# autonomousvision/unimatch

Hardware: AMD Instinct MI355X
Metric: image_pairs_per_sec (higher is better)
Workload: dtype f16x2

## Files before the change

### unimatch_amd/csrc/conv.hip

```cpp
#include <cstdlib>
#include <cstring>
#ifndef UM_CONV_2P
#define UM_CONV_2P 0
#endif
#include "common.h"
#include "planes.h"

struct ConvArgs {
    const unsigned short* ap;
    long a_plane_stride;
    unsigned row_stride;
    unsigned zero_row;
    const unsigned short* wp;
    long w_plane_stride;
    const float* bias;
    float* out;
    unsigned short* outp;
    long outp_plane_stride;
    int out_ld, out_coff, outp_ld, outp_coff;
    int act;
    int gate, gate_c, gate_zld;
    float* gate_h;
    const float* gate_z;
    float* gate_hout;
    int gate_hout_ld;
    float* stats;
    const float* addend;
    int addend_ld;
    int addend_period;
    int B, Hi, Wi, Cin, Ho, Wo, Cout;
    int KH, KW, stride, pad_h, pad_w;
    int M;
    float out_scale;
    int xcd;
    const float* xf;
    const float* nstats;
    int norm_relu;
};

__device__ __forceinline__ void conv_dma16(const void* base, unsigned byte_off, const unsigned char* lds_dst) {
    const unsigned dst = __builtin_amdgcn_readfirstlane(
        (unsigned)(unsigned long)(const __attribute__((address_space(3))) unsigned char*)lds_dst);
    unsigned keep;
    asm volatile("s_mov_b32 %0, m0\n\ts_mov_b32 m0, %3\n\ts_nop 0\n\tglobal_load_lds_dwordx4 %1, %2\n\ts_mov_b32 m0, %0"
                 : "=&s"(keep)
                 : "v"(byte_off), "s"(base), "s"(dst)
                 : "memory");
}

template <int V>
struct IntC {
    static constexpr int value = V;
};

template <typename T, int NS, int NT, int NT0, int NTP, int WSTRIDE, bool ADDEND>
__device__ __forceinline__ void conv_epilogue_pass(const ConvArgs& a, f32x16 (&acc)[NT], unsigned char* lds, unsigned char* scratch,
                                                   int bt, int rloc0, int nvalid, int part0, bool dense_parts, int n0, int tid,
                                                   int wave, int lane, int half) {
    const int P = a.Ho * a.Wo;
    constexpr int ROWB = 32 * NTP * 4;
    const int nb = n0 + 32 * NT0;
    unsigned char* stg = lds + wave * WSTRIDE;
    const int tl = lane & 31;
    constexpr int CPR = 8 * NTP;
    constexpr int ITER = 32 * CPR / 64;
    constexpr int BATCH = ITER < 4 ? ITER : 4, NBATCH = ITER / BATCH, NSIDE = NT == 4 ? 2 : 1;
    static_assert(ITER % BATCH == 0, "batches cover the iterations");
    const long rowbase = (long)bt * P + rloc0;
    const int nrows = nvalid;
    const int gate = a.gate;
    float* hbase = gate ? a.gate_h + rowbase * a.gate_c : nullptr;
    const float* zbase = gate == 2 ? a.gate_z + rowbase * a.gate_zld : nullptr;
    const float* abase = ADDEND && a.addend ? a.addend + rowbase * a.addend_ld : nullptr;
    const long aback = ADDEND && a.addend_period ? (long)bt * P * a.addend_ld : 0L;
    float* hobase = gate == 2 ? a.gate_hout + rowbase * a.gate_hout_ld : nullptr;
    f32x4 ad[NSIDE][BATCH], gz[NSIDE][BATCH], gh[NSIDE][BATCH];
    auto preload = [&](int b, int slot) {
        if (!abase && !gate) return;
#pragma unroll
        for (int j = 0; j < BATCH; ++j) {
            const int idx = (b * BATCH + j) * 64 + lane;
            const int r = idx / CPR, c = idx - r * CPR;
            const int col = nb + 4 * c;
            if (r < nrows && col < a.Cout) {
                if (abase) ad[slot][j] = *reinterpret_cast<const f32x4*>(abase - aback + (unsigned)(r * a.addend_ld + col));
                if (gate == 1 && col >= a.gate_c) gh[slot][j] = *reinterpret_cast<const f32x4*>(hbase + (unsigned)(r * a.gate_c + col - a.gate_c));
                if (gate == 2) {
                    gz[slot][j] = *reinterpret_cast<const f32x4*>(zbase + (unsigned)(r * a.gate_zld + col));
                    gh[slot][j] = *reinterpret_cast<const f32x4*>(hbase + (unsigned)(r * a.gate_c + col));
                }
            }
        }
    };
    preload(0, 0);
    auto to_lds = [&](auto act_tag, auto bias_tag) {
        constexpr int ACT = decltype(act_tag)::value;
        constexpr bool BIAS = decltype(bias_tag)::value != 0;
#pragma unroll
        for (int nt = 0; nt < NTP; ++nt)
#pragma unroll
            for (int g = 0; g < 4; ++g) {
                const int n = nb + 32 * nt + 8 * g + 4 * half;
                f32x4 v;
#pragma unroll
                for (int i = 0; i < 4; ++i) v[i] = acc[NT0 + nt][4 * g + i] * a.out_scale;
                if (BIAS) v = v + *reinterpret_cast<const f32x4*>(a.bias + min(n, a.Cout - 4));
#pragma unroll
                for (int i = 0; i < 4; ++i) {
                    if (ACT == 1) v[i] = fmaxf(v[i], 0.f);
                    else if (ACT == 2) v[i] = 1.0f / (1.0f + __expf(-v[i]));
                    else if (ACT == 3) v[i] = tanhf(v[i]);
                }
                const int c = 8 * nt + 2 * g + half;
                *reinterpret_cast<f32x4*>(stg + tl * ROWB + ((c ^ (tl & 7)) << 4)) = v;
            }
    };
    auto to_lds_b = [&](auto act_tag) {
        if (a.bias) to_lds(act_tag, IntC<1>{});
        else to_lds(act_tag, IntC<0>{});
    };
    switch (ADDEND && a.addend ? 0 : a.act) {
        case 0: to_lds_b(IntC<0>{}); break;
        case 1: to_lds_b(IntC<1>{}); break;
        case 2: to_lds_b(IntC<2>{}); break;
        default: to_lds_b(IntC<3>{}); break;
    }
    __builtin_amdgcn_wave_barrier();
    if (a.stats) {
        constexpr int RG = 64 / CPR >= 8 ? 8 : 64 / CPR >= 4 ? 4 : 2;
        constexpr int RPG = 32 / RG;
        const int nv = nvalid;
        const int c = lane % CPR, rg = lane / CPR;
        const f32x4 k = *reinterpret_cast<const f32x4*>(stg + (c << 4));
        f32x4 s1 = {0.f, 0.f, 0.f, 0.f}, s2 = {0.f, 0.f, 0.f, 0.f};
        if (rg < RG) {
            if (nv == 32) {
#pragma unroll
                for (int j = 0; j < RPG; ++j) {
                    const int r = rg * RPG + j;
                    const f32x4 d = *reinterpret_cast<const f32x4*>(stg + r * ROWB + ((c ^ (r & 7)) << 4)) - k;
                    s1 = s1 + d;
                    s2 = s2 + d * d;
                }
            } else {
#pragma unroll
                for (int j = 0; j < RPG; ++j) {
                    const int r = rg * RPG + j;
                    f32x4 d = *reinterpret_cast<const f32x4*>(stg + r * ROWB + ((c ^ (r & 7)) << 4)) - k;
                    if (r >= nv) d = f32x4{0.f, 0.f, 0.f, 0.f};
                    s1 = s1 + d;
                    s2 = s2 + d * d;
                }
            }
        }
#pragma unroll
        for (int step = CPR * RG / 2; step >= CPR; step >>= 1)
#pragma unroll
            for (int i = 0; i < 4; ++i) {
                s1[i] += __shfl_down(s1[i], step, 64);
                s2[i] += __shfl_down(s2[i], step, 64);
            }
        float* ws = reinterpret_cast<float*>(scratch) + wave * (2 * 32 * NT) + 32 * NT0;
        float* cnt = reinterpret_cast<float*>(scratch) + 8 * (2 * 32 * NT);
        if (lane == 0) cnt[wave] = (float)nv;
        if (lane < CPR) {
            const float inv = nv > 0 ? 1.0f / (float)nv : 0.f;
            *reinterpret_cast<f32x4*>(ws + 4 * c) = k + s1 * inv;
            *reinterpret_cast<f32x4*>(ws + 32 * NT + 4 * c) = s2 - s1 * s1 * inv;
        }
        __syncthreads();
        const int grp = tid >> 8, gt = tid & 255;
        if (gt < 32 * NTP && nb + gt < a.Cout && (cnt[4 * grp] > 0.f || dense_parts)) {
            const float* w0 = reinterpret_cast<const float*>(scratch) + grp * 4 * (2 * 32 * NT) + 32 * NT0;
            float mean = w0[gt], m2 = w0[32 * NT + gt];
            float n = cnt[4 * grp];
#pragma unroll
            for (int wv = 1; wv < 4; ++wv) {
                const float nw = cnt[4 * grp + wv];
                if (nw > 0.f) {
                    const float mw = w0[wv * (2 * 32 * NT) + gt], m2w = w0[wv * (2 * 32 * NT) + 32 * NT + gt];
                    const float delta = mw - mean, nn = n + nw;
                    mean += delta * (nw / nn);
                    m2 += m2w + delta * delta * (n * nw / nn);
                    n = nn;
                }
            }
            float* pr = a.stats + ((long)(part0 + grp) * 3) * a.Cout + nb + gt;
            pr[0] = n > 0.f ? mean : 0.f;
            pr[a.Cout] = n;
            pr[2 * a.Cout] = n > 0.f ? m2 : 0.f;
        }
    }
    auto store_rows = [&](auto gate_tag, auto add_tag) {
        constexpr int GATE = decltype(gate_tag)::value;
        constexpr bool ADD = decltype(add_tag)::value != 0;
        float* obase = a.out ? a.out + rowbase * a.out_ld + a.out_coff : nullptr;
        unsigned short* pbase = a.outp ? a.outp + rowbase * a.outp_ld + a.outp_coff : nullptr;
#pragma unroll
        for (int b = 0; b < NBATCH; ++b) {
            const int slot = NSIDE == 2 ? (b & 1) : 0;
            if ((ADD || GATE != 0) && NSIDE == 2 && b + 1 < NBATCH) preload(b + 1, (b + 1) & 1);
            if ((ADD || GATE != 0) && NSIDE == 1 && b > 0) preload(b, 0);
#pragma unroll
            for (int j = 0; j < BATCH; ++j) {
                const int idx = (b * BATCH + j) * 64 + lane;
                const int r = idx / CPR, c = idx - r * CPR;
                f32x4 d = *reinterpret_cast<const f32x4*>(stg + r * ROWB + ((c ^ (r & 7)) << 4));
                int col = nb + 4 * c;
                if (r < nrows && col < a.Cout) {
                    if (ADD) {
                        d = d + ad[slot][j];
#pragma unroll
                        for (int i = 0; i < 4; ++i) {
                            if (a.act == 1) d[i] = fmaxf(d[i], 0.f);
                            else if (a.act == 2) d[i] = 1.0f / (1.0f + __expf(-d[i]));
                            else if (a.act == 3) d[i] = tanhf(d[i]);
                        }
                    }
                    bool to_out = obase != nullptr, to_planes = pbase != nullptr;
                    if (GATE == 1) {
                        if (col >= a.gate_c) {
                            col -= a.gate_c;
                            d = d * gh[slot][j];
                            to_out = false;
                        } else {
                            to_planes = false;
                        }
                    } else if (GATE == 2) {
#pragma unroll
                        for (int i = 0; i < 4; ++i) d[i] = (1.0f - gz[slot][j][i]) * gh[slot][j][i] + gz[slot][j][i] * d[i];
                        *reinterpret_cast<f32x4*>(hobase + (unsigned)(r * a.gate_hout_ld + col)) = d;
                    }
                    if (to_out) __builtin_nontemporal_store(d, reinterpret_cast<f32x4*>(obase + (unsigned)(r * a.out_ld + col)));
                    if (to_planes) {
                        unsigned short* dst = pbase + (unsigned)(r * a.outp_ld + col);
                        const unsigned h0 = T::pack2(d[0], d[1]), h1 = T::pack2(d[2], d[3]);
                        *reinterpret_cast<u32x2*>(dst) = u32x2{h0, h1};
                        if (NS == 2) {
                            const f32x2 u0 = T::unpack2(h0), u1 = T::unpack2(h1);
                            const u32x2 lo = u32x2{T::pack2(d[0] - u0[0], d[1] - u0[1]), T::pack2(d[2] - u1[0], d[3] - u1[1])};
                            *reinterpret_cast<u32x2*>(dst + a.outp_plane_stride) = lo;
                        }
                    }
                }
            }
        }
    };
    auto store_rows_g = [&](auto gate_tag) {
        if (ADDEND && a.addend) store_rows(gate_tag, IntC<1>{});
        else store_rows(gate_tag, IntC<0>{});
    };
    if (a.gate == 0) store_rows_g(IntC<0>{});
    else if (a.gate == 1) store_rows_g(IntC<1>{});
    else store_rows_g(IntC<2>{});
}

template <typename T, int NS, int NT, int NTE = NT, bool ADDEND = true>
__device__ __forceinline__ void conv_epilogue(const ConvArgs& a, f32x16 (&acc)[NT], unsigned char* lds, unsigned char* scratch,
                                              int bt, int rloc0, int nvalid, int part0, bool dense_parts, int n0, int tid, int wave,
                                              int lane, int half) {
    constexpr int NP = NTE < NT ? NTE : NT;
    constexpr int WSTRIDE = 32 * (32 * NP * 4);
    conv_epilogue_pass<T, NS, NT, 0, NP, WSTRIDE, ADDEND>(a, acc, lds, scratch, bt, rloc0, nvalid, part0, dense_parts, n0, tid, wave, lane, half);
    if constexpr (NTE < NT)
        conv_epilogue_pass<T, NS, NT, NTE, NT - NTE, WSTRIDE, ADDEND>(a, acc, lds, scratch, bt, rloc0, nvalid, part0, dense_parts, n0, tid, wave,
                                                              lane, half);
}

struct ConvEntryArgs {
    const float* u;
    const float* ustats;
    const unsigned short* sp;
    long s_plane_stride;
    const unsigned short* wp2;
    long w2_plane_stride;
    const float* bias2;
    float* out2;
    float* stats2;
};

template <int NS, int NT>
struct ConvLds {
    static constexpr int TILE = 128 * 64;
    static constexpr int WTILE = 32 * NT * 64;
    static constexpr int STAGE = NS * (TILE + WTILE);
    static constexpr int EPI = 4 * 32 * (32 * NT * 4);
    static constexpr int RING = (2 * STAGE > EPI) ? 2 * STAGE : EPI;
    static constexpr int TOTAL = RING + 8 * 2 * 32 * NT * 4 + 64;
    static constexpr int ENTRY_CIN = 128;
    static constexpr int ENTRY_TOTAL = TOTAL + 2 * ENTRY_CIN * 4;
};

template <typename T, int NS, int NT, bool ENTRY>
__device__ __forceinline__ void conv_body(const ConvArgs& a, const ConvEntryArgs& e, unsigned char* lds) {
    using L = ConvLds<NS, NT>;
    constexpr int TILE = L::TILE, WTILE = L::WTILE, STAGE = L::STAGE, RING = L::RING;

    const int tid = threadIdx.x, lane = tid & 63;
    const int wave = __builtin_amdgcn_readfirstlane(tid >> 6);
    const int half = lane >> 5;
    const int P = a.Ho * a.Wo, tpi = (P + 127) / 128;
    const int ny = (a.Cout + 32 * NT - 1) / (32 * NT);
    const int wg = a.xcd ? xcd_remap(blockIdx.x, gridDim.x) : blockIdx.x;
    const int tile = wg / ny;
    const int bt = tile / tpi, pl0 = (tile - bt * tpi) * 128;
    const int n0 = (wg - tile * ny) * (32 * NT);
    const int cpt = a.Cin >> 5;
    const int nstage = a.KH * a.KW * cpt;
    const int ktot = a.KH * a.KW * a.Cin;

    const int dcp = lane & 3;
    int py[2], px[2], pbase[2];
    bool pok[2];
#pragma unroll
    for (int i = 0; i < 2; ++i) {
        const int p = pl0 + 32 * wave + 16 * i + (lane >> 2);
        pok[i] = p < P;
        const int rem = pok[i] ? p : 0;
        const int y = rem / a.Wo, x = rem - y * a.Wo;
        py[i] = y * a.stride - a.pad_h;
        px[i] = x * a.stride - a.pad_w;
        pbase[i] = bt * a.Hi * a.Wi;
    }
    const unsigned zero_row = a.zero_row;
    unsigned rowoff[2];
    auto set_tap = [&](int ky, int kx) {
#pragma unroll
        for (int i = 0; i < 2; ++i) {
            const int iy = py[i] + ky, ix = px[i] + kx;
            const bool ok = pok[i] && (unsigned)iy < (unsigned)a.Hi && (unsigned)ix < (unsigned)a.Wi;
            if constexpr (ENTRY) {
                rowoff[i] = ok ? (unsigned)(pbase[i] + iy * a.Wi + ix) : ~0u;
            } else {
                const unsigned row = ok ? (unsigned)(pbase[i] + iy * a.Wi + ix) : zero_row;
                rowoff[i] = row * a.row_stride;
            }
        }
    };
    int ky = 0, kx = 0, cc = 0;
    auto stage_async = [&](int c0, int kglob, unsigned char* buf) {
        if constexpr (!ENTRY) {
#pragma unroll
            for (int i = 0; i < 2; ++i) {
                const int r = 32 * wave + 16 * i + (lane >> 2);
                const int sc = dcp ^ ((r >> 2) & 3);
                const unsigned off = rowoff[i] + (unsigned)((c0 + 8 * sc) * 2);
#pragma unroll
                for (int pl = 0; pl < NS; ++pl) conv_dma16(a.ap + pl * a.a_plane_stride, off, buf + pl * TILE + (32 * wave + 16 * i) * 64);
            }
        }
#pragma unroll
        for (int i = 0; i < (2 * NT + 3) / 4; ++i) {
            const int j = wave + 4 * i;
            if (j < 2 * NT) {
                const int r = 16 * j + (lane >> 2);
                const int sc = dcp ^ ((r >> 2) & 3);
                const int n = min(n0 + r, a.Cout - 1);
                const unsigned off = (unsigned)(((long)n * ktot + kglob + 8 * sc) * 2);
#pragma unroll
                for (int pl = 0; pl < NS; ++pl)
                    conv_dma16(a.wp + pl * a.w_plane_stride, off, buf + NS * TILE + pl * WTILE + (16 * j) * 64);
            }
        }
    };
    const int esc = dcp ^ ((lane >> 4) & 3);
    float* sstat = reinterpret_cast<float*>(lds + L::TOTAL);
    f32x4 eu[2][2];
    u32x4 esh[2], esl[2];
    bool eok[2];
    int ec0 = 0;
    auto entry_load = [&](int c0) {
        ec0 = c0 + 8 * esc;
#pragma unroll
        for (int i = 0; i < 2; ++i) {
            eok[i] = rowoff[i] != ~0u;
            const unsigned el = (eok[i] ? rowoff[i] : 0u) * (unsigned)a.Cin + (unsigned)ec0;
            const unsigned char* pu = reinterpret_cast<const unsigned char*>(e.u) + el * 4u;
            eu[i][0] = *reinterpret_cast<const f32x4*>(pu);
            eu[i][1] = *reinterpret_cast<const f32x4*>(pu + 16);
            const unsigned char* ps = reinterpret_cast<const unsigned char*>(e.sp) + el * 2u;
            esh[i] = *reinterpret_cast<const u32x4*>(ps);
            if (NS == 2) esl[i] = *reinterpret_cast<const u32x4*>(ps + e.s_plane_stride * 2);
        }
    };
    auto entry_store = [&](unsigned char* buf) {
        float mu[8], rs[8];
        {
            const f32x4 m0 = *reinterpret_cast<const f32x4*>(sstat + ec0), m1 = *reinterpret_cast<const f32x4*>(sstat + ec0 + 4);
            const f32x4 r0 = *reinterpret_cast<const f32x4*>(sstat + a.Cin + ec0), r1 = *reinterpret_cast<const f32x4*>(sstat + a.Cin + ec0 + 4);
#pragma unroll
            for (int k = 0; k < 4; ++k) {
                mu[k] = m0[k];
                mu[4 + k] = m1[k];
                rs[k] = r0[k];
                rs[4 + k] = r1[k];
            }
        }
#pragma unroll
        for (int i = 0; i < 2; ++i) {
            float v[8], none[8];
#pragma unroll
            for (int k = 0; k < 4; ++k) {
                v[k] = eu[i][0][k];
                v[4 + k] = eu[i][1][k];
            }
#pragma unroll
            for (int k = 0; k < 8; ++k) none[k] = 0.f;
            u32x4 h, l = {0u, 0u, 0u, 0u};
            um_norm_value8<T, NS>(v, true, mu, rs, true, 2, none, false, none, none, esh[i], NS == 2 ? esl[i] : l, true, h, l);
            unsigned char* dst = buf + (32 * wave + 16 * i) * 64 + lane * 16;
#pragma unroll
            for (int k = 0; k < 4; ++k) {
                h[k] = eok[i] ? h[k] : 0u;
                l[k] = eok[i] ? l[k] : 0u;
            }
            *reinterpret_cast<u32x4*>(dst) = h;
            if (NS == 2) *reinterpret_cast<u32x4*>(dst + TILE) = l;
        }
    };

    f32x16 acc[NT];
#pragma unroll
    for (int nt = 0; nt < NT; ++nt)
#pragma unroll
        for (int r = 0; r < 16; ++r) acc[nt][r] = 0.f;
    f32x16 acc2[ENTRY ? NT : 1];
    if constexpr (ENTRY) {
#pragma unroll
        for (int nt = 0; nt < NT; ++nt)
#pragma unroll
            for (int r = 0; r < 16; ++r) acc2[nt][r] = 0.f;
    }

    const int fr = lane & 31;
    int foff[2];
#pragma unroll
    for (int ks = 0; ks < 2; ++ks) foff[ks] = fr * 64 + (((2 * ks + half) ^ ((fr >> 2) & 3)) << 4);

    i16x8 pwh[ENTRY ? NT : 1], pwl[ENTRY ? NT : 1];
    auto proj_load = [&](int pcc, int ks) {
#pragma unroll
        for (int nt = 0; nt < NT; ++nt) {
            const int n = min(n0 + 32 * nt + fr, a.Cout - 1);
            const unsigned short* pw = e.wp2 + (unsigned)(n * a.Cin + pcc * 32 + (2 * ks + half) * 8);
            pwh[nt] = *reinterpret_cast<const i16x8*>(pw);
            if (NS == 2) pwl[nt] = *reinterpret_cast<const i16x8*>(pw + e.w2_plane_stride);
        }
    };

    set_tap(0, 0);
    stage_async(0, 0, lds);
    if constexpr (ENTRY) {
        entry_load(0);
        for (int k = tid; k < 2 * a.Cin; k += 256) sstat[k] = e.ustats[(long)bt * 2 * a.Cin + k];
    }
    auto advance = [&]() {
        if (++cc == cpt) {
            cc = 0;
            if (++kx == a.KW) {
                kx = 0;
                ++ky;
            }
            set_tap(ky, kx);
        }
    };
    advance();
    if constexpr (ENTRY) {
        __syncthreads();
        entry_store(lds);
    }
    asm volatile("s_waitcnt vmcnt(0)" ::: "memory");
    __syncthreads();

    int ptap = 0, pcc = 0;
    for (int s = 0; s < nstage; ++s) {
        unsigned char* cur = lds + (s & 1) * STAGE;
        unsigned char* nxt = lds + ((s & 1) ^ 1) * STAGE;
        const bool centre = ENTRY && ptap == 4;
        if constexpr (ENTRY) {
            if (centre) proj_load(pcc, 0);
        }
        if (s + 1 < nstage) {
            stage_async(cc * 32, (s + 1) * 32, nxt);
            if constexpr (ENTRY) entry_load(cc * 32);
            advance();
        }
        const unsigned char* at = cur + 32 * wave * 64;
        const unsigned char* wt = cur + NS * TILE;
        __builtin_amdgcn_s_setprio(1);
#pragma unroll
        for (int ks = 0; ks < 2; ++ks) {
            const i16x8 bh = *reinterpret_cast<const i16x8*>(at + foff[ks]);
            i16x8 bl;
            if (NS == 2) bl = *reinterpret_cast<const i16x8*>(at + TILE + foff[ks]);
#pragma unroll
            for (int nt = 0; nt < NT; ++nt) {
                const i16x8 wh = *reinterpret_cast<const i16x8*>(wt + nt * 32 * 64 + foff[ks]);
                if (NS == 2) {
                    const i16x8 wl = *reinterpret_cast<const i16x8*>(wt + WTILE + nt * 32 * 64 + foff[ks]);
                    if (UM_CONV_2P != 1) acc[nt] = T::mfma(wl, bh, acc[nt]);
                    if (UM_CONV_2P != 2) acc[nt] = T::mfma(wh, bl, acc[nt]);
                }
                acc[nt] = T::mfma(wh, bh, acc[nt]);
            }
            if constexpr (ENTRY) {
                if (centre) {
#pragma unroll
                    for (int nt = 0; nt < NT; ++nt) {
                        if (NS == 2) {
                            if (UM_CONV_2P != 1) acc2[nt] = T::mfma(pwl[nt], bh, acc2[nt]);
                            if (UM_CONV_2P != 2) acc2[nt] = T::mfma(pwh[nt], bl, acc2[nt]);
                        }
                        acc2[nt] = T::mfma(pwh[nt], bh, acc2[nt]);
                    }
                    if (ks == 0) proj_load(pcc, 1);
                }
            }
        }
        __builtin_amdgcn_s_setprio(0);
        if constexpr (ENTRY) {
            if (s + 1 < nstage) entry_store(nxt);
            if (++pcc == cpt) {
                pcc = 0;
                ++ptap;
            }
        }
        asm volatile("s_waitcnt vmcnt(0)" ::: "memory");
        __syncthreads();
    }

    {
        const int rloc0 = pl0 + 32 * wave;
        conv_epilogue<T, NS, NT, NT, !ENTRY>(a, acc, lds, lds + RING, bt, rloc0, min(32, max(0, P - rloc0)), bt * ((P + 127) / 128) + pl0 / 128, false,
                                 n0, tid, wave, lane, half);
        if constexpr (ENTRY) {
            ConvArgs a2 = a;
            a2.bias = e.bias2;
            a2.out = e.out2;
            a2.stats = e.stats2;
            __syncthreads();
            conv_epilogue<T, NS, NT, NT, false>(a2, acc2, lds, lds + RING, bt, rloc0, min(32, max(0, P - rloc0)), bt * ((P + 127) / 128) + pl0 / 128,
                                     false, n0, tid, wave, lane, half);
        }
    }
}

template <typename T, int NS, int NT>
__global__ __launch_bounds__(256, 2) void conv_kernel(ConvArgs a) {
    __shared__ __attribute__((aligned(16))) unsigned char lds[ConvLds<NS, NT>::TOTAL];
    conv_body<T, NS, NT, false>(a, ConvEntryArgs{}, lds);
}

template <typename T, int NS, int NT>
__global__ __launch_bounds__(256, 2) void conv_entry_kernel(ConvArgs a, ConvEntryArgs e) {
    __shared__ __attribute__((aligned(16))) unsigned char lds[ConvLds<NS, NT>::ENTRY_TOTAL];
    conv_body<T, NS, NT, true>(a, e, lds);
}

template <int NS, int NT, int KW, int NSLOT>
struct ConvRowsLds {
    static constexpr int NTE = NT < 2 ? NT : 2;
    static constexpr int ATILE = 288 * 32;
    static constexpr int WTILE = 32 * NT * 32;
    static constexpr int STAGE = NS * (ATILE + KW * WTILE);
    static constexpr int EPI = 8 * 32 * (32 * NTE * 4);
    static constexpr int RING = (NSLOT * STAGE > EPI) ? NSLOT * STAGE : EPI;
    static constexpr int TOTAL = RING + 8 * 2 * 32 * NT * 4 + 64;
};

__device__ __forceinline__ void conv_wait_vm(int n) {
    switch (n) {
        case 0: asm volatile("s_waitcnt vmcnt(0)" ::: "memory"); break;
        case 1: asm volatile("s_waitcnt vmcnt(1)" ::: "memory"); break;
        case 2: asm volatile("s_waitcnt vmcnt(2)" ::: "memory"); break;
        case 3: asm volatile("s_waitcnt vmcnt(3)" ::: "memory"); break;
        case 4: asm volatile("s_waitcnt vmcnt(4)" ::: "memory"); break;
        case 6: asm volatile("s_waitcnt vmcnt(6)" ::: "memory"); break;
        case 8: asm volatile("s_waitcnt vmcnt(8)" ::: "memory"); break;
        case 9: asm volatile("s_waitcnt vmcnt(9)" ::: "memory"); break;
        case 12: asm volatile("s_waitcnt vmcnt(12)" ::: "memory"); break;
        case 16: asm volatile("s_waitcnt vmcnt(16)" ::: "memory"); break;
        case 18: asm volatile("s_waitcnt vmcnt(18)" ::: "memory"); break;
        case 24: asm volatile("s_waitcnt vmcnt(24)" ::: "memory"); break;
        default: asm volatile("s_waitcnt vmcnt(0)" ::: "memory"); break;
    }
}

template <typename T, int NS, int NT, int KW, int NSLOT>
__global__ __launch_bounds__(512, (NSLOT == 2 && NT < 4 ? 2 : 1)) void conv_rows_kernel(ConvArgs a) {
    using L = ConvRowsLds<NS, NT, KW, NSLOT>;
    constexpr int ATILE = L::ATILE, WTILE = L::WTILE, STAGE = L::STAGE, RING = L::RING;
    extern __shared__ __attribute__((aligned(16))) unsigned char lds[];

    const int tid = threadIdx.x, lane = tid & 63;
    const int wave = __builtin_amdgcn_readfirstlane(tid >> 6);
    const int half = lane >> 5, fr = lane & 31;
    const int P = a.Ho * a.Wo, tpi = (P + 255) / 256;
    const int ny = (a.Cout + 32 * NT - 1) / (32 * NT);
    const int wg = a.xcd ? xcd_remap(blockIdx.x, gridDim.x) : blockIdx.x;
    const int tile = wg / ny;
    const int bt = tile / tpi, pl0 = (tile - bt * tpi) * 256;
    const int n0 = (wg - tile * ny) * (32 * NT);
    const int cpt = a.Cin >> 4;
    const int nstage = a.KH * cpt;
    const int ktot = a.KH * KW * a.Cin;

    const int dcp = lane & 1;
    int wy[2];
    long wflat[2];
    bool wok[2];
#pragma unroll
    for (int i = 0; i < 2; ++i) {
        const int jr = i == 0 ? wave : 8;
        const int j = 32 * jr + (lane >> 1);
        const int p = pl0 + j - a.pad_w;
        wok[i] = (i == 0 || wave == 7) && p >= 0 && p < P;
        const int rem = wok[i] ? p : 0;
        wy[i] = rem / a.Wo - a.pad_h;
        wflat[i] = (long)bt * P + rem - (long)a.pad_h * a.Wi;
    }
    unsigned rowoff[2];
    auto set_ky = [&](int ky) {
#pragma unroll
        for (int i = 0; i < 2; ++i) {
            const int iy = wy[i] + ky;
            const bool ok = wok[i] && (unsigned)iy < (unsigned)a.Hi;
            const unsigned row = ok ? (unsigned)(wflat[i] + (long)ky * a.Wi) : a.zero_row;
            rowoff[i] = row * a.row_stride;
        }
    };
    constexpr int NPIECE = 2 + (KW * NT + 7) / 8;
    auto stage_piece = [&](int k, int ky, int cc, unsigned char* buf) {
        if (k < 2) {
            const int jr = k == 0 ? wave : 8;
            if (k == 0 || wave == 7) {
                const int r = 32 * jr + (lane >> 1);
                const int sc = dcp ^ ((r >> 3) & 1);
                const unsigned off = rowoff[k] + (unsigned)((cc * 16 + 8 * sc) * 2);
#pragma unroll
                for (int pl = 0; pl < NS; ++pl) conv_dma16(a.ap + pl * a.a_plane_stride, off, buf + pl * ATILE + (32 * jr) * 32);
            }
        } else {
            const int q = wave + 8 * (k - 2);
            if (q < KW * NT) {
                const int kx = q / NT, jb = q - kx * NT;
                const int r = 32 * jb + (lane >> 1);
                const int sc = dcp ^ ((r >> 3) & 1);
                const int n = min(n0 + r, a.Cout - 1);
                const unsigned off = (unsigned)(((long)n * ktot + (ky * KW + kx) * a.Cin + cc * 16 + 8 * sc) * 2);
#pragma unroll
                for (int pl = 0; pl < NS; ++pl)
                    conv_dma16(a.wp + pl * a.w_plane_stride, off, buf + NS * ATILE + (kx * NS + pl) * WTILE + (32 * jb) * 32);
            }
        }
    };

    bool tap_ok[KW];
    bool any_masked = false;
    {
        const int p = pl0 + 32 * wave + fr;
        const bool pok = p < P;
        const int x = (pok ? p : 0) % a.Wo;
#pragma unroll
        for (int kx = 0; kx < KW; ++kx) {
            tap_ok[kx] = pok && (unsigned)(x + kx - a.pad_w) < (unsigned)a.Wi;
            any_masked |= !tap_ok[kx];
        }
    }
    const bool wave_masked = __any(any_masked);

    f32x16 acc[NT];
#pragma unroll
    for (int nt = 0; nt < NT; ++nt)
#pragma unroll
        for (int r = 0; r < 16; ++r) acc[nt][r] = 0.f;

    const int foffw = fr * 32 + ((half ^ ((fr >> 3) & 1)) << 4);
    int foffa[KW];
#pragma unroll
    for (int kx = 0; kx < KW; ++kx) {
        const int r = 32 * wave + fr + kx;
        foffa[kx] = r * 32 + ((half ^ ((r >> 3) & 1)) << 4);
    }

    int cnt = NS * (1 + (wave == 7 ? 1 : 0));
#pragma unroll
    for (int k = 2; k < NPIECE; ++k) cnt += (wave + 8 * (k - 2) < KW * NT) ? NS : 0;
    constexpr int D = NSLOT - 1;

    int ky = 0, cc = 0;
    set_ky(0);
    auto advance = [&]() {
        if (++cc == cpt) {
            cc = 0;
            ++ky;
            set_ky(ky);
        }
    };
#pragma unroll
    for (int d = 0; d < D; ++d)
        if (d < nstage) {
#pragma unroll
            for (int k = 0; k < NPIECE; ++k) stage_piece(k, ky, cc, lds + d * STAGE);
            advance();
        }
    conv_wait_vm(nstage >= D ? cnt * (D - 1) : 0);
    __syncthreads();

    int cur_off = 0, nxt_off = D * STAGE;
    for (int s = 0; s < nstage; ++s) {
        unsigned char* cur = lds + cur_off;
        unsigned char* nxt = lds + nxt_off;
        const bool more = s + D < nstage;
        __builtin_amdgcn_s_setprio(1);
#pragma unroll
        for (int kx = 0; kx < KW; ++kx) {
            const unsigned char* wt = cur + NS * ATILE + kx * NS * WTILE;
            if (more) {
                constexpr int GROUPS = KW - 1;
#pragma unroll
                for (int k = 0; k < NPIECE; ++k)
                    if (k % GROUPS == kx && kx < GROUPS) stage_piece(k, ky, cc, nxt);
            }
            i16x8 bh = *reinterpret_cast<const i16x8*>(cur + foffa[kx]);
            i16x8 bl;
            if (NS == 2) bl = *reinterpret_cast<const i16x8*>(cur + ATILE + foffa[kx]);
            if (wave_masked && !tap_ok[kx]) {
                const i16x8 z = {0, 0, 0, 0, 0, 0, 0, 0};
                bh = z;
                bl = z;
            }
#pragma unroll
            for (int nt = 0; nt < NT; ++nt) {
                const i16x8 wh = *reinterpret_cast<const i16x8*>(wt + nt * 32 * 32 + foffw);
                if (NS == 2) {
                    const i16x8 wl = *reinterpret_cast<const i16x8*>(wt + WTILE + nt * 32 * 32 + foffw);
                    if (UM_CONV_2P != 1) acc[nt] = T::mfma(wl, bh, acc[nt]);
                    if (UM_CONV_2P != 2) acc[nt] = T::mfma(wh, bl, acc[nt]);
                }
                acc[nt] = T::mfma(wh, bh, acc[nt]);
            }
        }
        __builtin_amdgcn_s_setprio(0);
        if (more) advance();
        conv_wait_vm(more ? cnt * (D - 1) : 0);
        __syncthreads();
        cur_off = cur_off + STAGE == NSLOT * STAGE ? 0 : cur_off + STAGE;
        nxt_off = nxt_off + STAGE == NSLOT * STAGE ? 0 : nxt_off + STAGE;
    }
    {
        const int rloc0 = pl0 + 32 * wave;
        conv_epilogue<T, NS, NT, L::NTE>(a, acc, lds, lds + RING, bt, rloc0, min(32, max(0, P - rloc0)), bt * ((P + 127) / 128) + pl0 / 128,
                                         false, n0, tid, wave, lane, half);
    }
}


template <int NS, int NT>
struct ConvPatchLds {
    static constexpr int NTE = NT < 2 ? NT : 2;
    static constexpr int PW = 34, PPIX = 10 * PW;
    static constexpr int PROWS = 352;
    static constexpr int ATILE = PROWS * 32;
    static constexpr int WTILE = 32 * NT * 32;
    static constexpr int ASLOT = NS * ATILE, WSLOT = NS * 3 * WTILE;
    static constexpr int WBASE = 2 * ASLOT;
    static constexpr int STAGES = 2 * ASLOT + 2 * WSLOT;
    static constexpr int EPI = 8 * 32 * (32 * NTE * 4);
    static constexpr int SCRATCH = 8 * 2 * 32 * NT * 4 + 64;
    static constexpr int TOTAL = (STAGES > EPI + SCRATCH) ? STAGES : EPI + SCRATCH;
};

typedef const __attribute__((address_space(4))) float* um_const_f32p;

template <typename T, int NS, int NT, bool NORM>
__device__ __forceinline__ void conv_patch_body(const ConvArgs& a, unsigned char* lds) {
    using L = ConvPatchLds<NS, NT>;
    constexpr int ATILE = L::ATILE, WTILE = L::WTILE, ASLOT = L::ASLOT, WSLOT = L::WSLOT, WBASE = L::WBASE;
    constexpr int PW = L::PW;

    const int tid = threadIdx.x, lane = tid & 63;
    const int wave = __builtin_amdgcn_readfirstlane(tid >> 6);
    const int half = lane >> 5, fr = lane & 31;
    const int twn = (a.Wo + 31) >> 5, tpi = twn * ((a.Ho + 7) >> 3);
    const int ny = (a.Cout + 32 * NT - 1) / (32 * NT);
    const int wg = a.xcd ? xcd_remap(blockIdx.x, gridDim.x) : blockIdx.x;
    const int tile = wg / ny;
    const int bt = tile / tpi, tt = tile - bt * tpi;
    const int ty = tt / twn, tx = tt - ty * twn;
    const int y0 = ty * 8, x0 = tx * 32;
    const int n0 = (wg - tile * ny) * (32 * NT);
    const int cpt = a.Cin >> 4;
    const int ktot = 9 * a.Cin;

    const int dcp = lane & 1;
    unsigned rowoff[2];
#pragma unroll
    for (int i = 0; i < 2; ++i) {
        const int j = 32 * (wave + 8 * i) + (lane >> 1);
        const int py = j / PW, px = j - py * PW;
        const int iy = y0 - 1 + py, ix = x0 - 1 + px;
        const bool ok = j < L::PPIX && (unsigned)iy < (unsigned)a.Hi && (unsigned)ix < (unsigned)a.Wi;
        if constexpr (NORM) {
            rowoff[i] = ok ? (unsigned)((bt * a.Hi + iy) * a.Wi + ix) * (unsigned)(a.Cin * 4) : ~0u;
        } else {
            const unsigned row = ok ? (unsigned)((bt * a.Hi + iy) * a.Wi + ix) : a.zero_row;
            rowoff[i] = row * a.row_stride;
        }
    }
    auto stage_patch = [&](int cc, unsigned char* buf) {
#pragma unroll
        for (int i = 0; i < 2; ++i)
            if (i == 0 || wave < 3) {
                const int blk = wave + 8 * i;
                const int r = 32 * blk + (lane >> 1);
                const int sc = dcp ^ ((r >> 3) & 1);
                const unsigned off = rowoff[i] + (unsigned)((cc * 16 + 8 * sc) * 2);
#pragma unroll
                for (int pl = 0; pl < NS; ++pl) conv_dma16(a.ap + pl * a.a_plane_stride, off, buf + pl * ATILE + (32 * blk) * 32);
            }
    };
    const int nsc = dcp ^ ((lane >> 4) & 1);
    f32x4 nx0, nx1;
    auto norm_load = [&](int cc, int i) {
        const unsigned off = (rowoff[i] == ~0u ? 0u : rowoff[i]) + (unsigned)((cc * 16 + 8 * nsc) * 4);
        const unsigned char* p = reinterpret_cast<const unsigned char*>(a.xf) + off;
        nx0 = *reinterpret_cast<const f32x4*>(p);
        nx1 = *reinterpret_cast<const f32x4*>(p + 16);
    };
    auto norm_store = [&](int cc, int i, unsigned char* buf) {
        const um_const_f32p mu = (um_const_f32p)(unsigned long)(a.nstats + ((long)bt * 2) * a.Cin + cc * 16);
        const um_const_f32p rs = mu + a.Cin;
        float v[8];
#pragma unroll
        for (int k = 0; k < 8; ++k) {
            const float m = nsc ? mu[8 + k] : mu[k], r = nsc ? rs[8 + k] : rs[k];
            v[k] = ((k < 4 ? nx0[k & 3] : nx1[k & 3]) - m) * r;
        }
        if (a.norm_relu) {
#pragma unroll
            for (int k = 0; k < 8; ++k) v[k] = fmaxf(v[k], 0.f);
        }
        const bool ok = rowoff[i] != ~0u;
        u32x4 h = {T::pack2(v[0], v[1]), T::pack2(v[2], v[3]), T::pack2(v[4], v[5]), T::pack2(v[6], v[7])};
        unsigned char* dst = buf + (32 * (wave + 8 * i)) * 32 + lane * 16;
        if (NS == 2) {
            u32x4 l;
#pragma unroll
            for (int k = 0; k < 4; ++k) {
                const f32x2 u = T::unpack2(h[k]);
                l[k] = ok ? T::pack2(v[2 * k] - u[0], v[2 * k + 1] - u[1]) : 0u;
            }
            *reinterpret_cast<u32x4*>(dst + ATILE) = l;
        }
#pragma unroll
        for (int k = 0; k < 4; ++k) h[k] = ok ? h[k] : 0u;
        *reinterpret_cast<u32x4*>(dst) = h;
    };
    auto stage_w = [&](int cc, int ky, unsigned char* buf) {
#pragma unroll
        for (int k = 0; k < (3 * NT + 7) / 8; ++k) {
            const int q = wave + 8 * k;
            if (q < 3 * NT) {
                const int kx = q / NT, jb = q - kx * NT;
                const int r = 32 * jb + (lane >> 1);
                const int sc = dcp ^ ((r >> 3) & 1);
                const int n = min(n0 + r, a.Cout - 1);
                const unsigned off = (unsigned)(((long)n * ktot + (ky * 3 + kx) * a.Cin + cc * 16 + 8 * sc) * 2);
#pragma unroll
                for (int pl = 0; pl < NS; ++pl)
                    conv_dma16(a.wp + pl * a.w_plane_stride, off, buf + (kx * NS + pl) * WTILE + (32 * jb) * 32);
            }
        }
    };

    f32x16 acc[NT];
#pragma unroll
    for (int nt = 0; nt < NT; ++nt)
#pragma unroll
        for (int r = 0; r < 16; ++r) acc[nt][r] = 0.f;

    const int foffw = fr * 32 + ((half ^ ((fr >> 3) & 1)) << 4);
    int foffa[3][3];
#pragma unroll
    for (int ky = 0; ky < 3; ++ky)
#pragma unroll
        for (int kx = 0; kx < 3; ++kx) {
            const int r = (wave + ky) * PW + kx + fr;
            foffa[ky][kx] = r * 32 + ((half ^ ((r >> 3) & 1)) << 4);
        }

    if constexpr (NORM) {
        stage_w(0, 0, lds + WBASE);
        norm_load(0, 0);
        norm_store(0, 0, lds);
        if (wave < 3) {
            norm_load(0, 1);
            norm_store(0, 1, lds);
        }
    } else {
        stage_patch(0, lds);
        stage_w(0, 0, lds + WBASE);
    }
    asm volatile("s_waitcnt vmcnt(0)" ::: "memory");
    __syncthreads();

    for (int cc = 0; cc < cpt; ++cc) {
        const int a_cur = (cc & 1) * ASLOT, a_nxt = ASLOT - a_cur;
#pragma unroll
        for (int ky = 0; ky < 3; ++ky) {
            const int w_par = (cc + ky) & 1;
            const int w_cur = WBASE + w_par * WSLOT, w_nxt = WBASE + (w_par ^ 1) * WSLOT;
            const bool last = ky == 2 && cc + 1 == cpt;
            __builtin_amdgcn_s_setprio(1);
#pragma unroll
            for (int kx = 0; kx < 3; ++kx) {
                if (kx == 0 && !last) stage_w(ky == 2 ? cc + 1 : cc, ky == 2 ? 0 : ky + 1, lds + w_nxt);
                if constexpr (NORM) {
                    if (kx == 1 && cc + 1 < cpt) {
                        if (ky == 0) norm_load(cc + 1, 0);
                        if (ky == 1) {
                            norm_store(cc + 1, 0, lds + a_nxt);
                            if (wave < 3) norm_load(cc + 1, 1);
                        }
                        if (ky == 2 && wave < 3) norm_store(cc + 1, 1, lds + a_nxt);
                    }
                } else {
                    if (kx == 1 && ky == 0 && cc + 1 < cpt) stage_patch(cc + 1, lds + a_nxt);
                }
                const i16x8 bh = *reinterpret_cast<const i16x8*>(lds + a_cur + foffa[ky][kx]);
                i16x8 bl;
                if (NS == 2) bl = *reinterpret_cast<const i16x8*>(lds + a_cur + ATILE + foffa[ky][kx]);
                const unsigned char* wt = lds + w_cur + kx * NS * WTILE;
#pragma unroll
                for (int nt = 0; nt < NT; ++nt) {
                    const i16x8 wh = *reinterpret_cast<const i16x8*>(wt + nt * 32 * 32 + foffw);
                    if (NS == 2) {
                        const i16x8 wl = *reinterpret_cast<const i16x8*>(wt + WTILE + nt * 32 * 32 + foffw);
                        if (UM_CONV_2P != 1) acc[nt] = T::mfma(wl, bh, acc[nt]);
                        if (UM_CONV_2P != 2) acc[nt] = T::mfma(wh, bl, acc[nt]);
                    }
                    acc[nt] = T::mfma(wh, bh, acc[nt]);
                }
            }
            __builtin_amdgcn_s_setprio(0);
            asm volatile("s_waitcnt vmcnt(0)" ::: "memory");
            __syncthreads();
        }
    }
    const int nvalid = y0 + wave < a.Ho ? min(32, a.Wo - x0) : 0;
    conv_epilogue<T, NS, NT, L::NTE>(a, acc, lds, lds + L::EPI, bt, (y0 + wave) * a.Wo + x0, nvalid, (bt * tpi + tt) * 2, true, n0, tid,
                                     wave, lane, half);
}

template <typename T, int NS, int NT>
__global__ __launch_bounds__(512, (NT < 4 ? 2 : 1)) void conv_patch_kernel(ConvArgs a) {
    extern __shared__ __attribute__((aligned(16))) unsigned char lds[];
    conv_patch_body<T, NS, NT, false>(a, lds);
}

template <typename T, int NS, int NT>
__global__ __launch_bounds__(512, (NT < 4 ? 2 : 1)) void conv_patch_norm_kernel(ConvArgs a) {
    extern __shared__ __attribute__((aligned(16))) unsigned char lds[];
    conv_patch_body<T, NS, NT, true>(a, lds);
}

extern void um_set_error(const char* fmt, ...);

static int conv_xcd_enabled() {
    static const int on = um_debug_env("UM_CONV_NO_XCD") == nullptr;
    return on;
}

template <int NT>
static hipError_t launch_conv(const ConvArgs& a, int mode, hipStream_t stream) {
    dim3 grid(a.B * ((a.Ho * a.Wo + 127) / 128) * ((a.Cout + 32 * NT - 1) / (32 * NT))), block(256);
    ScopedKernelTimer timer(UM_K_CONV, stream);
    um_census_hit(UM_V_CONV_GENERIC);
    if (mode == 0)
        hipLaunchKernelGGL((conv_kernel<Fp16, 2, NT>), grid, block, 0, stream, a);
    else
        hipLaunchKernelGGL((conv_kernel<Bf16, 1, NT>), grid, block, 0, stream, a);
    return hipGetLastError();
}

template <int NT>
static hipError_t launch_conv_entry(const ConvArgs& a, const ConvEntryArgs& e, int mode, hipStream_t stream) {
    dim3 grid(a.B * ((a.Ho * a.Wo + 127) / 128) * ((a.Cout + 32 * NT - 1) / (32 * NT))), block(256);
    ScopedKernelTimer timer(UM_K_CONV, stream);
    um_census_hit(UM_V_CONV_GENERIC);
    if (mode == 0)
        hipLaunchKernelGGL((conv_entry_kernel<Fp16, 2, NT>), grid, block, 0, stream, a, e);
    else
        hipLaunchKernelGGL((conv_entry_kernel<Bf16, 1, NT>), grid, block, 0, stream, a, e);
    return hipGetLastError();
}

template <int NT, int KW, int NSLOT>
static hipError_t launch_conv_rows(const ConvArgs& a, int mode, hipStream_t stream) {
    static bool configured[2] = {false, false};
    dim3 grid(a.B * ((a.Ho * a.Wo + 255) / 256) * ((a.Cout + 32 * NT - 1) / (32 * NT))), block(512);
    constexpr int LDS2 = ConvRowsLds<2, NT, KW, NSLOT>::TOTAL, LDS1 = ConvRowsLds<1, NT, KW, NSLOT>::TOTAL;
    static_assert(LDS2 <= 160 * 1024 && LDS1 <= 160 * 1024, "ring beyond the CU's LDS");
    ScopedKernelTimer timer(UM_K_CONV, stream);
    um_census_hit(UM_V_CONV_ROWS);
    if (mode == 0) {
        if (!configured[0]) {
            hipError_t e = hipFuncSetAttribute(reinterpret_cast<const void*>(&conv_rows_kernel<Fp16, 2, NT, KW, NSLOT>),
                                               hipFuncAttributeMaxDynamicSharedMemorySize, LDS2);
            if (e != hipSuccess) return e;
            configured[0] = true;
        }
        hipLaunchKernelGGL((conv_rows_kernel<Fp16, 2, NT, KW, NSLOT>), grid, block, LDS2, stream, a);
    } else {
        if (!configured[1]) {
            hipError_t e = hipFuncSetAttribute(reinterpret_cast<const void*>(&conv_rows_kernel<Bf16, 1, NT, KW, NSLOT>),
                                               hipFuncAttributeMaxDynamicSharedMemorySize, LDS1);
            if (e != hipSuccess) return e;
            configured[1] = true;
        }
        hipLaunchKernelGGL((conv_rows_kernel<Bf16, 1, NT, KW, NSLOT>), grid, block, LDS1, stream, a);
    }
    return hipGetLastError();
}

template <int NT, bool NORM = false>
static hipError_t launch_conv_patch(const ConvArgs& a, int mode, hipStream_t stream) {
    static bool configured[2] = {false, false};
    dim3 grid(a.B * ((a.Ho + 7) / 8) * ((a.Wo + 31) / 32) * ((a.Cout + 32 * NT - 1) / (32 * NT))), block(512);
    constexpr int LDS2 = ConvPatchLds<2, NT>::TOTAL, LDS1 = ConvPatchLds<1, NT>::TOTAL;
    static_assert(LDS2 <= 160 * 1024 && LDS1 <= 160 * 1024, "ring beyond the CU's LDS");
    ScopedKernelTimer timer(UM_K_CONV, stream);
    um_census_hit(UM_V_CONV_PATCH);
    if (NORM) um_census_hit(UM_V_CONV_PATCH_NORM);
    void (*k2)(ConvArgs), (*k1)(ConvArgs);
    if constexpr (NORM) {
        k2 = conv_patch_norm_kernel<Fp16, 2, NT>;
        k1 = conv_patch_norm_kernel<Bf16, 1, NT>;
    } else {
        k2 = conv_patch_kernel<Fp16, 2, NT>;
        k1 = conv_patch_kernel<Bf16, 1, NT>;
    }
    if (mode == 0) {
        if (!configured[0]) {
            hipError_t e = hipFuncSetAttribute(reinterpret_cast<const void*>(k2), hipFuncAttributeMaxDynamicSharedMemorySize, LDS2);
            if (e != hipSuccess) return e;
            configured[0] = true;
        }
        hipLaunchKernelGGL(k2, grid, block, LDS2, stream, a);
    } else {
        if (!configured[1]) {
            hipError_t e = hipFuncSetAttribute(reinterpret_cast<const void*>(k1), hipFuncAttributeMaxDynamicSharedMemorySize, LDS1);
            if (e != hipSuccess) return e;
            configured[1] = true;
        }
        hipLaunchKernelGGL(k1, grid, block, LDS1, stream, a);
    }
    return hipGetLastError();
}

enum ConvKind { CONV_GENERIC = 0, CONV_ROWS = 1, CONV_PATCH = 2 };

static ConvKind conv_pick(int hi, int wi, int ho, int wo, int cout, int kh, int kw, int stride, int pad_h, int pad_w, int* nt_out) {
    const int nt = (cout % 128 == 0 || cout > 192) ? 4 : (cout % 96 == 0) ? 3 : (cout <= 64 || cout % 64 == 0) ? 2 : 4;
    *nt_out = nt;
    static const bool rows_enabled = um_debug_env("UM_CONV_NO_ROWS") == nullptr;
    static const char* patch_env = um_debug_env("UM_CONV_PATCH");
    static const char* patch_nts = patch_env ? patch_env : "234";
    const bool same = stride == 1 && ho == hi && wo == wi && (long)ho * wo >= 256 && rows_enabled;
    const bool rows3 = same && kw == 3 && pad_w == 1, rows5 = same && kw == 5 && pad_w == 2 && nt == 4;
    const long tiled = (long)((ho + 7) / 8 * 8) * ((wo + 31) / 32 * 32);
    if (rows3 && kh == 3 && pad_h == 1 && 4L * ho * wo >= 3 * tiled && strchr(patch_nts, '0' + nt) != nullptr) {
        if (cout <= 32) *nt_out = 1;
        return CONV_PATCH;
    }
    return rows3 || rows5 ? CONV_ROWS : CONV_GENERIC;
}

static constexpr bool kNormOnLoad[5] = {false, false, true, true, true};

extern "C" int um_conv2d_norm_supported(int hi, int wi, int cin, int cout, int kh, int kw, int stride, int pad_h, int pad_w, int mode) {
    if (hi <= 0 || wi <= 0 || cin <= 0 || cin % 32 != 0 || cout <= 0 || cout % 4 != 0 || kh <= 0 || kw <= 0 || stride <= 0 || pad_h < 0 ||
        pad_w < 0 || (mode != 0 && mode != 1))
        return 0;
    const int ho = (hi + 2 * pad_h - kh) / stride + 1, wo = (wi + 2 * pad_w - kw) / stride + 1;
    if (ho <= 0 || wo <= 0) return 0;
    int nt;
    if (conv_pick(hi, wi, ho, wo, cout, kh, kw, stride, pad_h, pad_w, &nt) != CONV_PATCH) return 0;
    return nt >= 2 && nt <= 4 && kNormOnLoad[nt] ? 1 : 0;
}

static constexpr bool kEntryConv[5] = {false, false, false, true, true};

extern "C" int um_conv2d_entry_supported(int hi, int wi, int cin, int cout, int kh, int kw, int stride, int pad_h, int pad_w, int mode) {
    if (hi <= 0 || wi <= 0 || cin <= 0 || cin % 32 != 0 || cin > ConvLds<2, 4>::ENTRY_CIN || cout <= 0 || cout % 4 != 0 ||
        (mode != 0 && mode != 1))
        return 0;
    if (kh != 3 || kw != 3 || stride != 2 || pad_h != 1 || pad_w != 1) return 0;
    const int ho = (hi - 1) / 2 + 1, wo = (wi - 1) / 2 + 1;
    int nt;
    if (conv_pick(hi, wi, ho, wo, cout, 3, 3, 2, 1, 1, &nt) != CONV_GENERIC) return 0;
    return nt >= 3 && nt <= 4 && kEntryConv[nt] ? 1 : 0;
}

extern "C" int um_conv_stats_parts(int hi, int wi, int cout, int kh, int kw, int stride, int pad_h, int pad_w) {
    if (hi <= 0 || wi <= 0 || cout <= 0 || kh <= 0 || kw <= 0 || stride <= 0 || pad_h < 0 || pad_w < 0) return -1;
    const int ho = (hi + 2 * pad_h - kh) / stride + 1, wo = (wi + 2 * pad_w - kw) / stride + 1;
    if (ho <= 0 || wo <= 0) return -1;
    int nt;
    if (conv_pick(hi, wi, ho, wo, cout, kh, kw, stride, pad_h, pad_w, &nt) == CONV_PATCH) return 2 * ((ho + 7) / 8) * ((wo + 31) / 32);
    return (int)(((long)ho * wo + 127) / 128);
}

static int conv2d_impl(const void* a_planes, int a_ld, int a_coff, long a_rows, const void* w_planes, const float* bias,
                       float* out, int out_ld, int out_coff, void* out_planes, int outp_ld, int outp_coff, long outp_rows,
                       float* stats_out, int batch, int hi, int wi, int cin, int cout, int kh, int kw, int stride,
                       int pad_h, int pad_w, int act, int wshift, int mode, void* stream_, int gate, float* gate_h,
                       const float* gate_z, int gate_zld, const float* addend = nullptr, int addend_ld = 0, float* gate_hout = nullptr,
                       int gate_hout_ld = 0, const float* norm_x = nullptr, const float* norm_stats = nullptr, int norm_relu = 0,
                       int addend_period = 0) {
// ... 434 lines not shown
```

Before: 957.2.

## Interleave conv weight/patch DMA issue with MFMA and precompute DMA addresses

```diff
diff --git a/unimatch_amd/csrc/conv.hip b/unimatch_amd/csrc/conv.hip
--- a/unimatch_amd/csrc/conv.hip
+++ b/unimatch_amd/csrc/conv.hip
@@ -3,8 +3,25 @@
 #ifndef UM_CONV_2P
 #define UM_CONV_2P 0
 #endif
+#ifndef UM_CONV_STAGE_LATE
+#define UM_CONV_STAGE_LATE 9
+#endif
 #include "common.h"
 #include "planes.h"
+
+#ifdef UM_CONV_TRACE
+__device__ unsigned long long* g_um_conv_trace = nullptr;
+#define UM_CSTAMP(stage, slot)                                                          \
+    do {                                                                                \
+        if (tracing && (stage) < 24) {                                                  \
+            __builtin_amdgcn_sched_barrier(0);                                          \
+            trace_buf[(stage) * 4 + (slot)] = __builtin_amdgcn_s_memtime();             \
+            __builtin_amdgcn_sched_barrier(0);                                          \
+        }                                                                               \
+    } while (0)
+#else
+#define UM_CSTAMP(stage, slot) do { } while (0)
+#endif
 
 struct ConvArgs {
     const unsigned short* ap;
@@ -48,6 +65,15 @@
                  : "memory");
 }
 
+__device__ __forceinline__ void conv_dma16_at(const void* base, unsigned byte_off, unsigned lds_addr) {
+    lds_addr = __builtin_amdgcn_readfirstlane(lds_addr);
+    unsigned keep;
+    asm volatile("s_mov_b32 %0, m0\n\ts_mov_b32 m0, %3\n\ts_nop 0\n\tglobal_load_lds_dwordx4 %1, %2\n\ts_mov_b32 m0, %0"
+                 : "=&s"(keep)
+                 : "v"(byte_off), "s"(base), "s"(lds_addr)
+                 : "memory");
+}
+
 template <int V>
 struct IntC {
     static constexpr int value = V;
@@ -310,6 +336,7 @@
     const int ktot = a.KH * a.KW * a.Cin;
 
     const int dcp = lane & 3;
+    const int esc = dcp ^ ((lane >> 4) & 3);
     int py[2], px[2], pbase[2];
     bool pok[2];
 #pragma unroll
@@ -333,37 +360,33 @@
                 rowoff[i] = ok ? (unsigned)(pbase[i] + iy * a.Wi + ix) : ~0u;
             } else {
                 const unsigned row = ok ? (unsigned)(pbase[i] + iy * a.Wi + ix) : zero_row;
-                rowoff[i] = row * a.row_stride;
+                rowoff[i] = row * a.row_stride + (unsigned)(16 * esc);
             }
         }
     };
     int ky = 0, kx = 0, cc = 0;
-    auto stage_async = [&](int c0, int kglob, unsigned char* buf) {
+    const unsigned lds0 = __builtin_amdgcn_readfirstlane((unsigned)(unsigned long)(const __attribute__((address_space(3))) unsigned char*)lds);
+    auto stage_async = [&](int c0, int kglob, unsigned slot) {
         if constexpr (!ENTRY) {
 #pragma unroll
-            for (int i = 0; i < 2; ++i) {
-                const int r = 32 * wave + 16 * i + (lane >> 2);
-                const int sc = dcp ^ ((r >> 2) & 3);
-                const unsigned off = rowoff[i] + (unsigned)((c0 + 8 * sc) * 2);
-#pragma unroll
-                for (int pl = 0; pl < NS; ++pl) conv_dma16(a.ap + pl * a.a_plane_stride, off, buf + pl * TILE + (32 * wave + 16 * i) * 64);
-            }
+            for (int i = 0; i < 2; ++i)
+#pragma unroll
+                for (int pl = 0; pl < NS; ++pl)
+                    conv_dma16_at(a.ap + pl * a.a_plane_stride + c0, rowoff[i], lds0 + slot + (unsigned)wave * 2048u + (unsigned)(pl * TILE + i * 1024));
         }
 #pragma unroll
         for (int i = 0; i < (2 * NT + 3) / 4; ++i) {
             const int j = wave + 4 * i;
             if (j < 2 * NT) {
-                const int r = 16 * j + (lane >> 2);
-                const int sc = dcp ^ ((r >> 2) & 3);
-                const int n = min(n0 + r, a.Cout - 1);
-                const unsigned off = (unsigned)(((long)n * ktot + kglob + 8 * sc) * 2);
+                const int n = min(n0 + 16 * j + (lane >> 2), a.Cout - 1);
+                const unsigned off = (unsigned)(((long)n * ktot + 8 * esc) * 2);
 #pragma unroll
                 for (int pl = 0; pl < NS; ++pl)
-                    conv_dma16(a.wp + pl * a.w_plane_stride, off, buf + NS * TILE + pl * WTILE + (16 * j) * 64);
-            }
-        }
-    };
-    const int esc = dcp ^ ((lane >> 4) & 3);
+                    conv_dma16_at(a.wp + pl * a.w_plane_stride + kglob, off,
+                                  lds0 + slot + (unsigned)wave * 1024u + (unsigned)(NS * TILE + pl * WTILE + i * 4096));
+            }
+        }
+    };
     float* sstat = reinterpret_cast<float*>(lds + L::TOTAL);
     f32x4 eu[2][2];
     u32x4 esh[2], esl[2];
@@ -449,7 +472,7 @@
     };
 
     set_tap(0, 0);
-    stage_async(0, 0, lds);
+    stage_async(0, 0, 0u);
     if constexpr (ENTRY) {
         entry_load(0);
         for (int k = tid; k < 2 * a.Cin; k += 256) sstat[k] = e.ustats[(long)bt * 2 * a.Cin + k];
@@ -477,12 +500,14 @@
         unsigned char* cur = lds + (s & 1) * STAGE;
         unsigned char* nxt = lds + ((s & 1) ^ 1) * STAGE;
         const bool centre = ENTRY && ptap == 4;
+        const bool more = s + 1 < nstage;
+        constexpr bool LATE = ((UM_CONV_STAGE_LATE >> (ENTRY ? 3 : 2)) & 1) != 0;
         if constexpr (ENTRY) {
+            if (more) entry_load(cc * 32);
             if (centre) proj_load(pcc, 0);
         }
-        if (s + 1 < nstage) {
-            stage_async(cc * 32, (s + 1) * 32, nxt);
-            if constexpr (ENTRY) entry_load(cc * 32);
+        if (!LATE && more) {
+            stage_async(cc * 32, (s + 1) * 32, (unsigned)(((s & 1) ^ 1) * STAGE));
             advance();
         }
         const unsigned char* at = cur + 32 * wave * 64;
@@ -502,6 +527,10 @@
                     if (UM_CONV_2P != 2) acc[nt] = T::mfma(wh, bl, acc[nt]);
                 }
                 acc[nt] = T::mfma(wh, bh, acc[nt]);
+            }
+            if (LATE && ks == 0 && more) {
+                stage_async(cc * 32, (s + 1) * 32, (unsigned)(((s & 1) ^ 1) * STAGE));
+                advance();
             }
             if constexpr (ENTRY) {
                 if (centre) {
@@ -805,19 +834,18 @@
             rowoff[i] = ok ? (unsigned)((bt * a.Hi + iy) * a.Wi + ix) * (unsigned)(a.Cin * 4) : ~0u;
         } else {
             const unsigned row = ok ? (unsigned)((bt * a.Hi + iy) * a.Wi + ix) : a.zero_row;
-            rowoff[i] = row * a.row_stride;
-        }
-    }
-    auto stage_patch = [&](int cc, unsigned char* buf) {
+            rowoff[i] = row * a.row_stride + (unsigned)(16 * (dcp ^ ((j >> 3) & 1)));
+        }
+    }
+    const unsigned lds_wave = __builtin_amdgcn_readfirstlane(
+        (unsigned)(unsigned long)(const __attribute__((address_space(3))) unsigned char*)lds) + (unsigned)wave * 1024u;
+    auto stage_patch = [&](int cc, int a_slot) {
 #pragma unroll
         for (int i = 0; i < 2; ++i)
             if (i == 0 || wave < 3) {
-                const int blk = wave + 8 * i;
-                const int r = 32 * blk + (lane >> 1);
-                const int sc = dcp ^ ((r >> 3) & 1);
-                const unsigned off = rowoff[i] + (unsigned)((cc * 16 + 8 * sc) * 2);
-#pragma unroll
-                for (int pl = 0; pl < NS; ++pl) conv_dma16(a.ap + pl * a.a_plane_stride, off, buf + pl * ATILE + (32 * blk) * 32);
+#pragma unroll
+                for (int pl = 0; pl < NS; ++pl)
+                    conv_dma16_at(a.ap + pl * a.a_plane_stride + cc * 16, rowoff[i], lds_wave + (unsigned)(a_slot + pl * ATILE + 8 * i * 1024));
             }
     };
     const int nsc = dcp ^ ((lane >> 4) & 1);
@@ -857,21 +885,26 @@
         for (int k = 0; k < 4; ++k) h[k] = ok ? h[k] : 0u;
         *reinterpret_cast<u32x4*>(dst) = h;
     };
-    auto stage_w = [&](int cc, int ky, unsigned char* buf) {
-#pragma unroll
-        for (int k = 0; k < (3 * NT + 7) / 8; ++k) {
-            const int q = wave + 8 * k;
-            if (q < 3 * NT) {
-                const int kx = q / NT, jb = q - kx * NT;
-                const int r = 32 * jb + (lane >> 1);
-                const int sc = dcp ^ ((r >> 3) & 1);
-                const int n = min(n0 + r, a.Cout - 1);
-                const unsigned off = (unsigned)(((long)n * ktot + (ky * 3 + kx) * a.Cin + cc * 16 + 8 * sc) * 2);
-#pragma unroll
-                for (int pl = 0; pl < NS; ++pl)
-                    conv_dma16(a.wp + pl * a.w_plane_stride, off, buf + (kx * NS + pl) * WTILE + (32 * jb) * 32);
-            }
-        }
+    constexpr int NKW = (3 * NT + 7) / 8, NPW = NS * NKW;
+    unsigned woff[NKW], wdst[NKW];
+#pragma unroll
+    for (int k = 0; k < NKW; ++k) {
+        const int q = min(wave + 8 * k, 3 * NT - 1);
+        const int kx = q / NT, jb = q - kx * NT;
+        const int r = 32 * jb + (lane >> 1);
+        const int sc = dcp ^ ((r >> 3) & 1);
+        const int n = min(n0 + r, a.Cout - 1);
+        woff[k] = (unsigned)(((long)n * ktot + kx * a.Cin + 8 * sc) * 2);
+        wdst[k] = lds_wave - (unsigned)wave * 1024u + (unsigned)(WBASE + kx * NS * WTILE + jb * 1024);
+    }
+    auto stage_w_piece = [&](int p, int cc, int ky, int w_slot) {
+        const int k = p / NS, pl = p - k * NS;
+        if (wave + 8 * k < 3 * NT)
+            conv_dma16_at(a.wp + pl * a.w_plane_stride + (ky * 3 * a.Cin + cc * 16), woff[k], wdst[k] + (unsigned)(w_slot + pl * WTILE));
+    };
+    auto stage_w = [&](int cc, int ky, int w_slot) {
+#pragma unroll
+        for (int p = 0; p < NPW; ++p) stage_w_piece(p, cc, ky, w_slot);
     };
 
     f32x16 acc[NT];
@@ -890,8 +923,13 @@
             foffa[ky][kx] = r * 32 + ((half ^ ((r >> 3) & 1)) << 4);
         }
 
+#ifdef UM_CONV_TRACE
+    const bool tracing = g_um_conv_trace != nullptr && (blockIdx.x % 37) == 0 && lane == 0 && (wave & 3) == 0;
+    unsigned long long* trace_buf = g_um_conv_trace + ((size_t)(blockIdx.x / 37) * 2 + (wave >> 2)) * (24 * 4 + 4);
+    if (tracing) trace_buf[24 * 4] = __builtin_amdgcn_s_memtime();
+#endif
     if constexpr (NORM) {
-        stage_w(0, 0, lds + WBASE);
+        stage_w(0, 0, 0);
         norm_load(0, 0);
         norm_store(0, 0, lds);
         if (wave < 3) {
@@ -899,25 +937,32 @@
             norm_store(0, 1, lds);
         }
     } else {
-        stage_patch(0, lds);
-        stage_w(0, 0, lds + WBASE);
+        stage_patch(0, 0);
+        stage_w(0, 0, 0);
     }
     asm volatile("s_waitcnt vmcnt(0)" ::: "memory");
     __syncthreads();
 
-    for (int cc = 0; cc < cpt; ++cc) {
-        const int a_cur = (cc & 1) * ASLOT, a_nxt = ASLOT - a_cur;
+    auto chunk = [&](int cc, auto par_tag) {
+        constexpr int PARC = decltype(par_tag)::value;
+        constexpr bool LATE = ((UM_CONV_STAGE_LATE >> (NORM ? 1 : 0)) & 1) != 0;
+        const int PAR = PARC >= 0 ? PARC : (cc & 1);
+        const int a_cur = PAR * ASLOT, a_nxt = ASLOT - a_cur;
+        const bool more = cc + 1 < cpt;
 #pragma unroll
         for (int ky = 0; ky < 3; ++ky) {
-            const int w_par = (cc + ky) & 1;
-            const int w_cur = WBASE + w_par * WSLOT, w_nxt = WBASE + (w_par ^ 1) * WSLOT;
-            const bool last = ky == 2 && cc + 1 == cpt;
+            const int w_par = (PAR + ky) & 1;
+            const int w_cur = WBASE + w_par * WSLOT, w_nxt = (w_par ^ 1) * WSLOT;
+            const bool next_w = ky < 2 || more;
+            const int kx_w = (NORM || ky == 0) ? 2 : 1;
+            UM_CSTAMP(3 * cc + ky, 0);
+            if (!LATE && next_w) stage_w(ky == 2 ? cc + 1 : cc, ky == 2 ? 0 : ky + 1, w_nxt);
+            const int npos = (3 - kx_w) * NT;
             __builtin_amdgcn_s_setprio(1);
 #pragma unroll
             for (int kx = 0; kx < 3; ++kx) {
-                if (kx == 0 && !last) stage_w(ky == 2 ? cc + 1 : cc, ky == 2 ? 0 : ky + 1, lds + w_nxt);
                 if constexpr (NORM) {
-                    if (kx == 1 && cc + 1 < cpt) {
+                    if (kx == 1 && more) {
                         if (ky == 0) norm_load(cc + 1, 0);
                         if (ky == 1) {
                             norm_store(cc + 1, 0, lds + a_nxt);
@@ -926,7 +971,7 @@
                         if (ky == 2 && wave < 3) norm_store(cc + 1, 1, lds + a_nxt);
                     }
                 } else {
-                    if (kx == 1 && ky == 0 && cc + 1 < cpt) stage_patch(cc + 1, lds + a_nxt);
+                    if (kx == 1 && ky == 0 && more) stage_patch(cc + 1, a_nxt);
                 }
                 const i16x8 bh = *reinterpret_cast<const i16x8*>(lds + a_cur + foffa[ky][kx]);
                 i16x8 bl;
@@ -941,16 +986,41 @@
                         if (UM_CONV_2P != 2) acc[nt] = T::mfma(wh, bl, acc[nt]);
                     }
                     acc[nt] = T::mfma(wh, bh, acc[nt]);
+                    if (kx == 0 && nt == 0) UM_CSTAMP(3 * cc + ky, 1);
+                    if (LATE && kx >= kx_w && next_w) {
+                        const int pos = (kx - kx_w) * NT + nt;
+#pragma unroll
+                        for (int p = 0; p < NPW; ++p)
+                            if (p * npos / NPW == pos) stage_w_piece(p, ky == 2 ? cc + 1 : cc, ky == 2 ? 0 : ky + 1, w_nxt);
+                    }
                 }
             }
             __builtin_amdgcn_s_setprio(0);
+            UM_CSTAMP(3 * cc + ky, 2);
             asm volatile("s_waitcnt vmcnt(0)" ::: "memory");
+            UM_CSTAMP(3 * cc + ky, 3);
             __syncthreads();
         }
-    }
+    };
+    if constexpr (NORM) {
+        for (int cc = 0; cc < cpt; ++cc) chunk(cc, IntC<-1>{});
+    } else {
+        int cc = 0;
+        for (; cc + 1 < cpt; cc += 2) {
+            chunk(cc, IntC<0>{});
+            chunk(cc + 1, IntC<1>{});
+        }
+        if (cc < cpt) chunk(cc, IntC<0>{});
+    }
+#ifdef UM_CONV_TRACE
+    if (tracing) trace_buf[24 * 4 + 1] = __builtin_amdgcn_s_memtime();
+#endif
     const int nvalid = y0 + wave < a.Ho ? min(32, a.Wo - x0) : 0;
     conv_epilogue<T, NS, NT, L::NTE>(a, acc, lds, lds + L::EPI, bt, (y0 + wave) * a.Wo + x0, nvalid, (bt * tpi + tt) * 2, true, n0, tid,
                                      wave, lane, half);
+#ifdef UM_CONV_TRACE
+    if (tracing) trace_buf[24 * 4 + 2] = __builtin_amdgcn_s_memtime();
+#endif
 }
 
 template <typename T, int NS, int NT>
@@ -966,6 +1036,11 @@
 }
 
 extern void um_set_error(const char* fmt, ...);
+#ifdef UM_CONV_TRACE
+extern "C" int um_debug_set_conv_trace(void* ptr) {
+    return (int)hipMemcpyToSymbol(HIP_SYMBOL(g_um_conv_trace), &ptr, sizeof(ptr));
+}
+#endif
 
 static int conv_xcd_enabled() {
     static const int on = um_debug_env("UM_CONV_NO_XCD") == nullptr;
```

After: 958.8, median of 6. No clear change (+0.2%).
